# Pixel-Talk/CanonSwap

Hardware: AMD Instinct MI355X
Metric: frames/sec at 512x512 (generator hot path F->W->T->R->W->G) (higher is better)
Workload: dtype f16; 1 GPU; BASELINE configs[2]: 512x512 video, 64 frames batched per launch on each GPU, steady state over 1280 frames (20 launches per GPU) (256x256 crops in, random-init weights of the real architecture); frames_per_launch_per_gpu=64, frames_total=1280, parallelism=frame-shard x1, identities_resident=1, latency_mode=False, accumulate=fp32, debug_decodes=False

## Files before the change

canonswap_amd/csrc/conv_epilogue.h:

```cpp
#pragma once
#include "common.h"

#ifndef EP_TL
#define EP_TL(i) do { } while (0)
#endif
typedef unsigned int ep_u4_t __attribute__((ext_vector_type(4)));
typedef unsigned int ep_u2_t __attribute__((ext_vector_type(2)));

static inline int ep_check_extents(const ConvParams& p, const char* who)
{
    auto span = [&](const TDesc& t) -> long {
        return (long)(p.N - 1) * t.sN + (long)(p.D - 1) * t.sD + (long)(p.H - 1) * t.sH + (long)(p.W - 1) * t.sW + p.Cout;
    };
    auto wide = [&](const TDesc& t) { return t.sD >= (1L << 23) || t.sH >= (1L << 23) || t.sW >= (1L << 23); };
    const long lim = 1L << 31;
    long ph_max = 0;
    for (int z = 0; z < p.nphase && z < 4; ++z) ph_max = p.ph_ooff[z] > ph_max ? (long)p.ph_ooff[z] : ph_max;
    if ((p.out0.p && span(p.out0) + ph_max >= lim) || (p.out1.p && span(p.out1) >= lim) || (p.res.p && span(p.res) >= lim)) {
        cs_set_error("%s: a tensor of this launch spans 2^31 elements or more (32-bit in-tensor offsets)", who);
        return -1;
    }
    if ((p.out0.p && wide(p.out0)) || (p.out1.p && wide(p.out1)) || (p.res.p && wide(p.res)) || p.D >= (1 << 22) || p.H >= (1 << 22) ||
        p.W >= (1 << 22)) {
        cs_set_error("%s: an axis stride of 2^23 elements or more (24-bit multiplies in the addressing)", who);
// ... 78 lines not shown
__device__ __forceinline__ constexpr int ep_chan(int pair, int cstep, int wave_row0, int ci, int l4)
{
    if (pair == 1) return wave_row0 + (ci >> 1) * 32 + l4 * 8 + (ci & 1) * 4;
    if (pair == 2) return wave_row0 / 2 + (ci >> 2) * 32 + l4 * 8 + ((ci >> 1) & 1) * 4;
    const int pb = wave_row0 / 16 + ci;
    return (cstep == 2 ? (pb >> 1) : pb) * 16 + l4 * 4;
}
__device__ __forceinline__ constexpr bool ep_second(int pair, int ci) { return pair == 1 ? (ci & 1) != 0 : pair == 2 ? ((ci >> 1) & 1) != 0 : false; }
__device__ __forceinline__ bool ep_al8(const TDesc& t)
{
    return (((unsigned long long)t.p & 15ull) == 0) && (((t.sN | t.sD | t.sH | t.sW) & 7) == 0);
}
__device__ __forceinline__ constexpr int ep_pair_of(int mode, int wch)
{
    return (mode == MODE_PIXSHUF) ? 0 : (mode == MODE_TBLEND || mode == MODE_SPADE) ? (wch % 4 == 0 ? 2 : 0) : (wch % 2 == 0 ? 1 : 0);
}

#if defined(CS_EP_NOSTORE)
#define EP_STORE_COND && (p.N < 0)
#else
#define EP_STORE_COND
#endif
#define CONV_EPILOGUE_EARLY_FETCH() \
    ep_u2_t ep_xpre[EP_EARLY ? EP_WPX0 : 1][EP_EARLY ? (WCH + 1) / 2 : 1]; \
    if constexpr (EP_EARLY) { \
        int xlw, xlh, xld, xln; \
        { int t = l15p; xlw = t & mW; t >>= lgTW; xlh = t & mH; t >>= lgTH; xld = t & mD; t >>= lgTD; xln = t; } \
        const int xrs = p.res_shift, xnb = tn * (BM >> lgS); \
        const unsigned xlane = (unsigned)((xnb + xln) * (int)p.res.sN + __mul24((td << lgTD) + xld, (int)p.res.sD) + \
                                          __mul24(((th << lgTH) + xlh) >> xrs, (int)p.res.sH) + __mul24(((tw << lgTW) + xlw) >> xrs, (int)p.res.sW)); \
_Pragma("unroll") \
        for (int pi = 0; pi < EP_WPX0; ++pi) { \
            int bw, bh, bd, bn; \
            { int t = (ep_wpx0 * EP_WPX0 + pi) << 4; bw = t & mW; t >>= lgTW; bh = t & mH; t >>= lgTH; bd = t & mD; t >>= lgTD; bn = t; } \
            const unsigned xb = xlane + (unsigned)(bn * (int)p.res.sN + bd * (int)p.res.sD + (bh >> xrs) * (int)p.res.sH + (bw >> xrs) * (int)p.res.sW); \
_Pragma("unroll") \
            for (int ci = 0; ci < WCH; ci += 2) { \
                const int cb = ep_chan(EP_PAIR, 2, n0 + wch * WCH * 16, ci, l4); \
                ep_u2_t q2; q2[0] = 0u; q2[1] = 0u; \
                if (p.res.p && xnb + xln + bn < p.N && cb < p.Cout) q2 = *(const ep_u2_t*)((const half_t*)p.res.p + (xb + (unsigned)cb)); \
                ep_xpre[pi][ci / 2] = q2; \
            } \
        } \
    }

template <int N> __device__ __forceinline__ float ep_row_shl(float a)
{
#ifdef EP_HOST_EMULATION
    (void)a;
    return 0.f;
#else
    return __builtin_bit_cast(float, __builtin_amdgcn_update_dpp(0, __builtin_bit_cast(int, a), 0x100 | N, 0xf, 0xf, true));
#endif
}

__device__ __forceinline__ float ep_row_sum16(float a)
{
#ifdef EP_HOST_EMULATION
    for (int o = 1; o < 16; o <<= 1) a += __shfl_xor(a, o, 64);
    return a;
#else
    a += __builtin_bit_cast(float, __builtin_amdgcn_update_dpp(0, __builtin_bit_cast(int, a), 0x101, 0xf, 0xf, true));
    a += __builtin_bit_cast(float, __builtin_amdgcn_update_dpp(0, __builtin_bit_cast(int, a), 0x102, 0xf, 0xf, true));
    a += __builtin_bit_cast(float, __builtin_amdgcn_update_dpp(0, __builtin_bit_cast(int, a), 0x104, 0xf, 0xf, true));
    a += __builtin_bit_cast(float, __builtin_amdgcn_update_dpp(0, __builtin_bit_cast(int, a), 0x108, 0xf, 0xf, true));
    return a;
#endif
}

#define EP_STAT_FLUSH(sg) \
    if (EP_STAT) { \
        const int ep_tiles = p.nTW * p.nTH * p.nTD; \
        const int ep_nblk = EP_NBLK_V; \
        const int ep_blk = EP_BLK_V(sg); \
_Pragma("unroll") \
        for (int ci = 0; ci < WCH; ci += CSTEP) { \
            const int cb = ep_chan(EP_PAIR, CSTEP, n0 + wch * WCH * 16, ci, l4); \
            float ep_pa[4], ep_pb[4]; \
_Pragma("unroll") \
            for (int r = 0; r < 4; ++r) { \
                ep_pa[r] = ep_row_sum16(ep_sum[EP_STAT ? ci : 0][r]); ep_pb[r] = ep_row_sum16(ep_sq[EP_STAT ? ci : 0][r]); \
                ep_sum[EP_STAT ? ci : 0][r] = 0.f; ep_sq[EP_STAT ? ci : 0][r] = 0.f; \
            } \
             \
            if (l15 == 0 && cb < p.Cout) { \
                float4* dst = (float4*)(p.stat_out + (((long)tn * ep_nblk + ep_blk) * p.Cout + cb) * 2); \
                dst[0] = make_float4(ep_pa[0], ep_pb[0], ep_pa[1], ep_pb[1]); \
                dst[1] = make_float4(ep_pa[2], ep_pb[2], ep_pa[3], ep_pb[3]); \
            } \
        } \
    }

#ifndef EP_GSEL_V
#define EP_GSEL_V 0
#endif
#ifndef EP_BLK_V
#define EP_BLK_V(sg) ((tile_lin % ep_tiles) * (BM / (EP_SG * 16)) + ep_wpx * (EP_WPX / EP_SG) + (sg))
#define EP_NBLK_V (ep_tiles * (BM / (EP_SG * 16)))
#endif
#ifndef EP_SLICE_FENCE
#define EP_SLICE_FENCE
#endif
#ifndef EP_FG
#define EP_FG 8
#endif
#ifndef EP_FG_F32
#define EP_FG_F32 4
#endif
#ifndef EP_FG_STAT
#define EP_FG_STAT 4
#endif
#ifndef EP_PIPE_V
#define EP_PIPE_V 0
#endif
#ifndef EP_O0_EXTRA_V
#define EP_O0_EXTRA_V 0u
#endif
#ifndef EP_POOL_WSH_V
#define EP_POOL_WSH_V 0
#define EP_POOL_HSH_V 0
#endif
#define EP_POOLB 128
#ifndef EP_SPMUL_V
#define EP_SPMUL_V 0
#endif
#ifndef EP_O1ONLY_V
#define EP_O1ONLY_V 0
#endif
#ifndef EP_MLIN_V
#define EP_MLIN_V 0
#endif
#ifndef EP_DUP_V
#define EP_DUP_V 0
#endif
#define EP_SPMULB 256
#define EP_GELUB 512
#define EP_FETCH_ROUND(PG0, BI) \
    if (EP_PF && !EP_EARLY && (ep_fetch || ep_has_ps)) { \
_Pragma("unroll") \
        for (int g = 0; g < EP_G; ++g) { \
            int bw, bh, bd, bn; \
            { int t = (ep_wpx * EP_WPX + (PG0) + g) << 4; bw = t & mW; t >>= lgTW; bh = t & mH; t >>= lgTH; bd = t & mD; t >>= lgTD; bn = t; } \
            if (!EPFAST && ep_nb + ep_ln + bn >= p.N) continue; \
            if (ep_has_ps) ep_ps2[BI][g] = p.pixscale[ep_lane_ps + (unsigned)((((bn * p.D + bd) * p.H + bh) * p.W + bw) * p.ps_stride)]; \
            if (ep_fetch) { \
                const unsigned xb = ep_lane_res + (unsigned)(bn * (int)p.res.sN + bd * (int)p.res.sD + (bh >> ep_rs) * (int)p.res.sH + \
                                                            (bw >> ep_rs) * (int)p.res.sW); \
_Pragma("unroll") \
                for (int ci = 0; ci < WCH; ci += CSTEP) { \
                    const int cb = ep_chan(EP_PAIR, CSTEP, n0 + wch * WCH * 16, ci, l4); \
                    if (!EPALL && cb >= p.Cout) continue; \
                    if (ep_res32) ep_raw2[BI][g][(EP_PF ? ci / CSTEP : 0)] = *(const ep_u4_t*)((const float*)p.res.p + (xb + (unsigned)cb)); \
                    else if (ep_mr && ep_second(EP_PAIR, ci)) {  } \
                    else if (ep_mr && (EPALL || cb + 4 < p.Cout)) ep_raw2[BI][g][(EP_PF ? ci / CSTEP : 0)] = *(const ep_u4_t*)((const half_t*)p.res.p + (xb + (unsigned)cb)); \
                    else { \
                        const ep_u2_t q2 = *(const ep_u2_t*)((const half_t*)p.res.p + (xb + (unsigned)cb)); \
                        ep_raw2[BI][g][(EP_PF ? ci / CSTEP : 0)][0] = q2[0]; ep_raw2[BI][g][(EP_PF ? ci / CSTEP : 0)][1] = q2[1]; \
                    } \
                } \
            } \
        } \
    }
#define CONV_EPILOGUE_IMPL(EPCODE) \
    constexpr int EPF = (EPCODE); \
    constexpr bool EPFAST = EPF >= 0; \
    constexpr bool EPALL = EPFAST && ((EPF >> 6) & 1) == 0;       \
    constexpr bool EP_POOL = EPFAST && ((EPF >> 7) & 1) != 0 && (EP_POOL_WSH_V) > 0;       \
    constexpr int EP_PS = EP_POOL ? 1 : 0; \
    constexpr bool EP_GELU = EPFAST && ((EPF >> 9) & 1) != 0;           \
    const bool ep_spm = EPFAST ? (((EPF >> 8) & 1) != 0) : ((MODE == MODE_STD) && p.spmul != 0); \
    constexpr bool EP_POOL_HB = EP_POOL && (EP_POOL_HSH_V) == 0;       \
    float ep_phold[EP_POOL_HB ? WCH : 1][4];                            \
    const bool ep_has_res = EPFAST ? ((EPF & 3) != 0) : (p.res.p != nullptr); \
    const bool ep_res32 = EPFAST ? ((EPF & 3) == 2) : (p.res_f32 != 0); \
    const bool ep_has_o0 = EPFAST ? (((EPF >> 2) & 1) != 0) : (p.out0.p != nullptr); \
// ... 43 lines not shown
    { int t = l15p; ep_lw = t & mW; t >>= lgTW; ep_lh = t & mH; t >>= lgTH; ep_ld = t & mD; t >>= lgTD; ep_ln = t; } \
    const int ep_w0 = tw << lgTW, ep_h0 = th << lgTH, ep_d0 = td << lgTD, ep_nb = tn * (BM >> lgS); \
    const int ep_rs = (MODE == MODE_SPADE || ep_spm) ? p.res_shift : 0; \
     \
    const bool ep_tn1 = (BM >> lgS) == 1; \
    const unsigned ep_lane_res = (unsigned)(ep_nb * (int)p.res.sN + (ep_tn1 ? 0 : ep_ln * (int)p.res.sN) + __mul24(ep_d0 + ep_ld, (int)p.res.sD) + \
                                            __mul24((ep_h0 + ep_lh) >> ep_rs, (int)p.res.sH) + __mul24((ep_w0 + ep_lw) >> ep_rs, (int)p.res.sW)); \
    const unsigned ep_lane_o0 = (EP_O0_EXTRA_V) + (unsigned)(ep_nb * (int)p.out0.sN + (ep_tn1 ? 0 : ep_ln * (int)p.out0.sN) + __mul24(ep_d0 + ep_ld, (int)p.out0.sD) + \
                                           __mul24((ep_h0 + ep_lh) >> EP_PS, (int)p.out0.sH) + __mul24((ep_w0 + ep_lw) >> EP_PS, (int)p.out0.sW)); \
     \
    const bool ep_pool_lane = !EP_POOL || (lane & ((EP_POOL_WSH_V) | (EP_POOL_HSH_V))) == 0; \
    const unsigned ep_lane_o1 = (EP_O0_EXTRA_V) + (unsigned)(ep_nb * (int)p.out1.sN + (ep_tn1 ? 0 : ep_ln * (int)p.out1.sN) + __mul24(ep_d0 + ep_ld, (int)p.out1.sD) + \
                                           __mul24(ep_h0 + ep_lh, (int)p.out1.sH) + __mul24(ep_w0 + ep_lw, (int)p.out1.sW)); \
    const unsigned ep_lane_ps = (unsigned)(((((ep_nb + ep_ln) * p.D + ep_d0 + ep_ld) * p.H + ep_h0 + ep_lh) * p.W + ep_w0 + ep_lw) * p.ps_stride); \
     \
    const unsigned ep_lane_px = (unsigned)((((ep_nb + ep_ln) * 3) * 2 * p.H + 2 * (ep_h0 + ep_lh)) * 2 * p.W + 2 * (ep_w0 + ep_lw)); \
     \
    constexpr bool EP_PIPE = (EP_PIPE_V) != 0 && EP_G < EP_WPX; \
    ep_u4_t ep_raw2[EP_PIPE ? 2 : 1][EP_G][EP_NCI]; float ep_ps2[EP_PIPE ? 2 : 1][EP_G]; \
    if (EP_PIPE) { EP_FETCH_ROUND(0, 0) } \
_Pragma("unroll") \
    for (int pg = 0; pg < EP_WPX; pg += EP_G) { \
    const int ep_bi = EP_PIPE ? ((pg / EP_G) & 1) : 0; \
    if (!EP_PIPE) { EP_FETCH_ROUND(pg, 0) } \
    else if (pg + EP_G < EP_WPX) { EP_FETCH_ROUND(pg + EP_G, EP_PIPE ? (((pg / EP_G) + 1) & 1) : 0) } \
    ep_u4_t (&ep_raw)[EP_G][EP_NCI] = ep_raw2[ep_bi]; float (&ep_ps)[EP_G] = ep_ps2[ep_bi]; \
    if (pg == 0) EP_TL(6); \
_Pragma("unroll") \
    for (int g = 0; g < EP_G; ++g) { \
        const int pi = pg + g; \
        if (pi == 1) EP_TL(7); \
        if (pi > 0 && pi % EP_SG == 0) { EP_STAT_FLUSH(pi / EP_SG - 1) } \
        int bw, bh, bd, bn; \
        { int t = (ep_wpx * EP_WPX + pi) << 4; bw = t & mW; t >>= lgTW; bh = t & mH; t >>= lgTH; bd = t & mD; t >>= lgTD; bn = t; } \
        if (!EPFAST && ep_nb + ep_ln + bn >= p.N) continue; \
        float ps = 1.f; \
        if (ep_has_ps) ps = EP_PF ? ep_ps[g] : p.pixscale[ep_lane_ps + (unsigned)((((bn * p.D + bd) * p.H + bh) * p.W + bw) * p.ps_stride)]; \
        const unsigned xb = ep_lane_res + (unsigned)(bn * (int)p.res.sN + bd * (int)p.res.sD + (bh >> ep_rs) * (int)p.res.sH + (bw >> ep_rs) * (int)p.res.sW); \
        const unsigned ob0 = ep_lane_o0 + (unsigned)(bn * (int)p.out0.sN + bd * (int)p.out0.sD + (bh >> EP_PS) * (int)p.out0.sH + (bw >> EP_PS) * (int)p.out0.sW); \
        const unsigned ob1 = ep_lane_o1 + (unsigned)(bn * (int)p.out1.sN + bd * (int)p.out1.sD + bh * (int)p.out1.sH + bw * (int)p.out1.sW); \
        float ep_vh[4] = {0.f, 0.f, 0.f, 0.f}, ep_uh[4] = {0.f, 0.f, 0.f, 0.f};       \
_Pragma("unroll") \
        for (int ci = 0; ci < WCH; ci += CSTEP) { \
            const int cb = ep_chan(EP_PAIR, CSTEP, n0 + wch * WCH * 16, ci, l4); \
            if (!EPALL && cb >= p.Cout) continue; \
            float rr[4] = {0.f, 0.f, 0.f, 0.f};      \
            if (ep_has_res) { \
                if (EP_EARLY) { \
                    const h4_t hx = __builtin_bit_cast(h4_t, ep_xpre[EP_EARLY ? pi : 0][EP_EARLY ? ci / 2 : 0]); \
_Pragma("unroll") \
                    for (int r = 0; r < 4; ++r) rr[r] = (float)hx[r]; \
                } else if (EP_PF) { \
                    const bool ep_hi = ep_mr && ep_second(EP_PAIR, ci);       \
                    const ep_u4_t q4 = ep_raw[g][(EP_PF ? ci / CSTEP : 0)]; \
                    const ep_u4_t qp = ep_raw[g][(EP_PF && ep_second(EP_PAIR, ci) ? ci / CSTEP - 1 : 0)]; \
                    if (ep_res32) { \
                        const f4_t qf = __builtin_bit_cast(f4_t, q4);      \
_Pragma("unroll") \
                        for (int r = 0; r < 4; ++r) rr[r] = qf[r]; \
                    } else { \
                        ep_u2_t q2; q2[0] = ep_hi ? qp[2] : q4[0]; q2[1] = ep_hi ? qp[3] : q4[1]; \
                        const h4_t hx = __builtin_bit_cast(h4_t, q2); \
_Pragma("unroll") \
                        for (int r = 0; r < 4; ++r) rr[r] = (float)hx[r]; \
                    } \
                } else { \
                    load4(p.res, ep_res32, (long)(xb + (unsigned)cb), rr); \
// ... 155 lines not shown
```

canonswap_amd/csrc/conv_halo_kernel.h:

```cpp
#pragma once
#include <type_traits>
#include <utility>
#include <cstdlib>
#include "common.h"
#ifdef CS_TIMELINE
#define EP_TL(i) TL_STAMP(i)
#endif
#define EP_POOL_WSH_V EP_POOL_WSH_K
#define EP_POOL_HSH_V EP_POOL_HSH_K
#define EP_SPMUL_V EP_SPMUL_K
#define EP_DUP_V EP_DUP_K
#define EP_MLIN_V EP_MLIN_K
#define EP_O1ONLY_V EP_O1ONLY_K
#define EP_O0_EXTRA_V ep_o0_extra
#include "conv_epilogue.h"

typedef unsigned int u4_t __attribute__((ext_vector_type(4)));
__device__ __forceinline__ unsigned mdiv(unsigned u, unsigned magic) { return magic ? __umulhi(u, magic) : u; }

template <int OFF>
__device__ __forceinline__ void wfrag_load(u4_t& dst, const half_t* ptr)
{
    asm volatile("global_load_dwordx4 %0, %1, off offset:%2" : "=v"(dst) : "v"(ptr), "n"(OFF));
}
template <int N>
__device__ __forceinline__ void wait_vmcnt_le()
{
    asm volatile("s_waitcnt vmcnt(%0)" ::"n"(N) : "memory");
}

#ifdef CS_TIMELINE
extern unsigned long long* g_cs_tl;
extern long g_cs_tl_cap;
#define TL_STAMP(i) do { __builtin_amdgcn_sched_barrier(0); tl_t[i] = __builtin_amdgcn_s_memtime(); __builtin_amdgcn_sched_barrier(0); } while (0)
#else
#define TL_STAMP(i) do { } while (0)
#endif

template <int ST> struct StaticShape { static constexpr int KD = 0, KH = 0, KW = 0, LW = 0, LH = 0, LD = 0; };
template <> struct StaticShape<1> { static constexpr int KD = 1, KH = 3, KW = 3, LW = 4, LH = 3, LD = 0; };
template <> struct StaticShape<2> { static constexpr int KD = 3, KH = 3, KW = 3, LW = 3, LH = 3, LD = 1; };
template <> struct StaticShape<3> { static constexpr int KD = 3, KH = 3, KW = 3, LW = 2, LH = 2, LD = 4; };
template <> struct StaticShape<4> { static constexpr int KD = 7, KH = 7, KW = 1, LW = 3, LH = 3, LD = 1; };
template <> struct StaticShape<5> { static constexpr int KD = 3, KH = 3, KW = 3, LW = 2, LH = 2, LD = 3; };
template <> struct StaticShape<6> { static constexpr int KD = 7, KH = 7, KW = 1, LW = 1, LH = 3, LD = 3; };
template <> struct StaticShape<7> { static constexpr int KD = 3, KH = 3, KW = 3, LW = 3, LH = 3, LD = 2; };
template <> struct StaticShape<8> { static constexpr int KD = 7, KH = 7, KW = 1, LW = 1, LH = 3, LD = 4; };
// ... 9 lines not shown

template <int CK, int WPX, int WCH, int WVP, int ST, int MODE> constexpr int halo_pad()
{
#ifdef CS_LDS_V1
    return 1;
#else
    if (CK == 64 && WCH == 4 && WPX == 8 && ST == 1) return 2;
    if (CK == 32 && WCH == 5 && WPX == 8 && (ST == 7 || ST == 8 || ST == 9)) return 2;
    if (CK == 64 && WCH == 2 && WPX == 8 && WVP == 2 && ST == 16) return 2;
    if (CK == 32 && WCH == 2 && WPX == 8 && ST == 1 && MODE == MODE_SPADE) return 2;
#ifdef CS_LDS_V32
    if (CK == 32 && WCH == 2 && WPX == 4 && WVP == 4 && ST == 3) return 2;
#endif
    return 1;
#endif
}
template <int ST, int PAD> constexpr int halo_hi()
{
    if (PAD == 2) return ST == 3 ? 16 : (ST == 9 ? 19 : ((ST == 7 || ST == 8) ? 15 : (ST == 16 ? 13 : 8)));
    return ST == 4 ? 18 : ((ST == 3 || ST == 7 || ST == 8 || ST == 9) ? 13 : (ST == 12 ? 9 : 8));
}
template <int ST, int PAD> __host__ __device__ constexpr int halo_lane_pos(int l)
{
#ifdef CS_LDS_V1
    return l;
#else
    using SS = StaticShape<ST>;
    if (ST == 0 || SS::KW != 3 || SS::LW > 3 || SS::LW < 2) return l;
    if (SS::LW == 2 && PAD == 2) return ((l & 1) << 1) | ((l & 2) << 2) | ((l >> 2) & 1) | ((l & 8) >> 1);
    return ((l & 1) << 1) | ((l & 2) << 1) | ((l >> 2) & 1) | (l & 8);
#endif
}

template <class F, int... I> __device__ __forceinline__ void halo_static_for_impl(F&& f, std::integer_sequence<int, I...>) { (f(std::integral_constant<int, I>{}), ...); }
template <int N, class F> __device__ __forceinline__ void halo_static_for(F&& f) { halo_static_for_impl(static_cast<F&&>(f), std::make_integer_sequence<int, N>{}); }

template <int WCH, int PFS, int HI, int ST0>
constexpr int halo_ring_young(int st, int L, int NP, bool dma_cur)
{
    auto dma = [&](int u, bool on) { return (on && u >= ST0 && u < ST0 + HI) ? 1 : 0; };
    auto cur_before = [&](int from_step ) {
        int n = 0;
        for (int u = from_step; u < st; ++u) n += (u >= 1 ? WCH : 0) + dma(u, dma_cur);
        return n;
    };
    if (st >= PFS) {
        const int u0 = st - PFS + 1;
        return dma(u0, dma_cur) + cur_before(u0 + 1);
    }
    const int prime = (PFS - 1 - st) * WCH + cur_before(0);
    int g = 0;
    if (NP % PFS == 0) g = st + NP - PFS + 1;
    else { for (int u = NP - PFS + 1; u <= NP; ++u) if ((u - 1) % PFS == st) g = u; }
    int carried = dma(g, true);
    for (int u = g + 1; u <= NP; ++u) carried += WCH + (u < NP ? dma(u, true) : 0);
    carried += cur_before(0);
    return prime < carried ? prime : carried;
}

template <int ST, int PAD> constexpr int halo_pool_shift(int bit)
{
    for (int b = 0; b < 4; ++b) if (halo_lane_pos<ST, PAD>(1 << b) == (1 << bit)) return 1 << b;
    return 0;
}

template <int WCH, int ST> constexpr bool halo_phase_group() { return !(ST == 0 && WCH >= 4); }
// ... 41 lines not shown
    unsigned long long tl_t[8] = {0, 0, 0, 0, 0, 0, 0, 0};
    const unsigned long long tl_real0 = __builtin_amdgcn_s_memrealtime();
    TL_STAMP(0);
#endif

#ifdef CS_DEPHASE
    if (MODE == MODE_SPADE && WCH == 4) {
        unsigned hwid;
        asm volatile("s_getreg_b32 %0, hwreg(HW_REG_HW_ID)" : "=s"(hwid));
        if ((hwid & 1u) && (int)(blockIdx.x + blockIdx.y * gridDim.x) < 512)
            for (int i = 0; i < CS_DEPHASE; ++i) __builtin_amdgcn_s_sleep(16);
    }
#endif
    const int tid = threadIdx.x, lane = tid & 63;
    const int wave = __builtin_amdgcn_readfirstlane(tid >> 6);
    constexpr bool PHK = halo_phase_group<WCH, ST>();
    const int phz = (PHK && p.nphase) ? (int)blockIdx.z : 0;
    const int PHv = (PHK && p.nphase) ? p.ph_PH[phz] : p.PH, PWv = (PHK && p.nphase) ? p.ph_PW[phz] : p.PW;
    const unsigned ep_o0_extra = (PHK && p.nphase) ? p.ph_ooff[phz] : 0u;
    const int wpx = SK ? 0 : wave % WVP, wch = SK ? 0 : wave / WVP;
    const int l15 = lane & 15, l4 = lane >> 4;
    const int l15p = halo_lane_pos<ST, PAD>(l15);
#ifdef CS_NO_PAIR
    constexpr int EP_PAIR = 0;
#else
    constexpr int EP_PAIR = ep_pair_of(MODE, WCH);
#endif

#ifdef CS_NO_ASMRING
    constexpr bool ASMRK = false;
#else
    constexpr bool ASMRK = DB && !SK && CK == 32 && WCH == 5 && WPX == 8 && WVP == 2 && (ST == 7 || ST == 8 || ST == 9) && MODE == MODE_STD;
#endif
    u4_t wr_p[ASMRK ? 3 : 1][ASMRK ? WCH : 1];
    unsigned poffb[ASMRK ? HI : 1];
    __amdgpu_buffer_rsrc_t rsrc_p;
    int gbuf = 0;
    bool staged = false;
    const bool persist = ASMRK && p.persist_total > 0;
    int p_base = 0, p_cnt = 0, p_j = 0, p_i = 0, p_per = 1;
    if (persist) {
        const int total = p.persist_total, G = (int)gridDim.x;
        const int xcd = blockIdx.x & 7, q = total >> 3, r = total & 7;
        p_i = blockIdx.x >> 3; p_per = G >> 3;
        p_base = xcd * q + (xcd < r ? xcd : r); p_cnt = q + (xcd < r ? 1 : 0);
        if (p_i >= p_cnt) return;
    }
    for (;;) {
    int tile_lin = blockIdx.x, cblk = blockIdx.y;
    const bool has_next = persist && p_i + p_per * (p_j + 1) < p_cnt;
    auto u_to_tile = [&](int u, int& tl_, int& cb_) {
        const int ncb = p.Cout_pad / BN;
        tl_ = (int)mdiv((unsigned)u, p.mg_ncb); cb_ = u - tl_ * ncb;
    };
    if (persist) u_to_tile(p_base + p_i + p_per * p_j, tile_lin, cblk);
    else if (p.xcd_map != 0) {
        const int flat = p.xcd_map == 2;
        const int total = (int)gridDim.x;
        const int xcd = blockIdx.x & 7, i = blockIdx.x >> 3;
        const int q = total >> 3, r = total & 7;
        const int u = xcd * q + (xcd < r ? xcd : r) + i;
        if (flat) u_to_tile(u, tile_lin, cblk);
        else tile_lin = u;
    }
    int t = tile_lin, tq;
    tq = (int)mdiv((unsigned)t, p.mg_tw); const int tw = t - tq * p.nTW; t = tq;
// ... 46 lines not shown
    auto stage_halo = [&](int buf, int c0) {
        long coff = c0;
        int climit = p.Cin - c0;
        if ((CK == 32 || ST == 15 || (ST == 0 && WCH != 4)) && p.cg > 0) {
            const int j = c0 >> 5;
            coff = (long)(j / p.cg) * p.in_sG + (j % p.cg) * 32;
            climit = p.cg_cin - (j % p.cg) * 32;
        }
        if (pre) {
#pragma unroll
            for (int j = 0; j < HI; ++j) {
                const int q = tid + 256 * j;
                if (q < nitems) {
                    const bool ok = ((pmask >> j) & 1u) && ((q % SLP) * 8 < climit);
                    glds(ok ? p.in + poff[j] + coff : p.zero, buf, 256 * j + wave * 64);
                }
            }
        } else if constexpr (!DB) {
            for (int q0 = 0; q0 < nitems; q0 += 256) {
                const int q = q0 + tid;
                if (q < nitems) {
                    bool inb;
                    const int o = piece_off(q, inb);
                    const bool ok = inb && ((q % SLP) * 8 < climit);
                    glds(ok ? p.in + o + coff : p.zero, buf, q0 + wave * 64);
                }
            }
        }
    };

    int abase[WPX];
#pragma unroll
    for (int pi = 0; pi < WPX; ++pi) {
        int m = wpx * WPX * 16 + pi * 16 + l15p;
        const int wl = m & mW; m >>= lgTW;
        const int hl = m & mH; m >>= lgTH;
        const int dl = m & mD; m >>= lgTD;
        abase[pi] = (((m * HD + dl) * HH + hl) * HW + wl) * VS + l4 * 16;
    }
    const int nck = (p.Cin + CK - 1) / CK;
    const int j0 = SK ? wave : 0;
    int cc_lo = 0, cc_hi = nck;
    if (p.sk_out) { cc_lo = (int)(((long)nck * blockIdx.z) / gridDim.z); cc_hi = (int)(((long)nck * (blockIdx.z + 1)) / gridDim.z); }

    const half_t* wbase = p.wgt;
    if (p.wslot) wbase += p.wofs[p.wslot[nb < p.N ? nb : p.N - 1]];
    if (PHK && p.nphase) wbase += p.ph_wofs[phz];
    const half_t* wlane = wbase + ((long)(n0 + wch * WCH * 16) * 32 + ep_lane_row(EP_PAIR, l15) * 32 + l4 * 8);
    const long wstep = (long)p.Cout_pad * 32;

#ifdef CS_NO_EARLY
    constexpr bool EP_EARLY = false;
#else
    constexpr bool EP_EARLY = (MODE == MODE_SPADE) && !SK && ST != 0 && WCH == 2 && WPX == 8;
#endif
#ifdef CS_NO_EPFAST
    constexpr bool EP_FAST = false;
#else
    constexpr bool EP_FAST = !SK && ST != 0 && (WCH == 4 || WCH == 5 || (WCH == 2 && WPX == 8) || ST == 15);
#endif
    constexpr int EP_WPX0 = WPX;
    const int ep_wpx0 = wpx;
    CONV_EPILOGUE_EARLY_FETCH()

    f4_t acc[WCH][WPX];
#pragma unroll
    for (int ci = 0; ci < WCH; ++ci)
// ... 52 lines not shown
                const int climit = (nxt && !has_next) ? 0 : p.Cin - c0;
                const unsigned off = (((tid + 256 * j) % SLP) * 8 < climit) ? poffb[j] : OOB;
                __builtin_amdgcn_raw_ptr_buffer_load_lds(rsrc_p, (__attribute__((address_space(3))) void*)(smem + (size_t)buf * HSTRIDE + (size_t)(256 * j + wave * 64) * 16),
                                                         16, (int)off, c0 * 2, 0, 0);
            };
            auto wsrc_of = [&](int cc, int st, int nsc) -> const half_t* {
                int c2 = cc, s2 = st;
                if (st >= nsc) { c2 = cc + 1; s2 = (nsc % PFS == 0) ? st - nsc : (st - PFS) % PFS; }
                const int ccl = c2 < cc_hi ? c2 : cc_lo;
                return wlane + (long)(ccl * NT + s2) * wstep;
            };
            auto wload1 = [&](u4_t& dst, const half_t* src, int ci) {
                if (ci == 0) asm volatile("global_load_dwordx4 %0, %1, off" : "=v"(dst) : "v"(src));
                else if (ci == 1) asm volatile("global_load_dwordx4 %0, %1, off offset:1024" : "=v"(dst) : "v"(src));
                else if (ci == 2) asm volatile("global_load_dwordx4 %0, %1, off offset:2048" : "=v"(dst) : "v"(src));
                else if (ci == 3) asm volatile("global_load_dwordx4 %0, %1, off offset:3072" : "=v"(dst) : "v"(src));
                else asm volatile("global_load_dwordx4 %0, %1, off" : "=v"(dst) : "v"(src + 4 * 16 * 32));
            };
            static_assert(EP_PAIR == 0, "ASMR: plain weight row order");
            TL_STAMP(1);
            constexpr bool CARRY = ST != 9;
            if (!staged) {
                set_stage(nb, d0, h0, w0);
#pragma unroll
                for (int j = 0; j < HI; ++j) stage_piece(gbuf, cc_lo, j);
            }
            if (!staged || !CARRY) {
#pragma unroll
                for (int st = 0; st < PFS; ++st)
#pragma unroll
                    for (int ci = 0; ci < WCH; ++ci) wload1(wr[st][ci], wsrc_of(cc_lo, st, NS), ci);
            }
            TL_STAMP(2);
            auto run_chunk_a = [&](int cc, auto rag_t) {
                constexpr bool RAG = decltype(rag_t)::value;
                wait_vmcnt_le<PFS * WCH>();
                __builtin_amdgcn_s_barrier();
                asm volatile("" ::: "memory");
                const unsigned char* hb = smem + (size_t)gbuf * HSTRIDE;
                const int nbuf = gbuf ^ 1;
                gbuf ^= 1;
                if (cc + 1 == cc_hi && has_next) {
                    int ntl, ncb_, t2 = 0, q2;
                    u_to_tile(p_base + p_i + p_per * (p_j + 1), ntl, ncb_);
                    t2 = ntl;
                    q2 = (int)mdiv((unsigned)t2, p.mg_tw); const int tw2 = t2 - q2 * p.nTW; t2 = q2;
                    q2 = (int)mdiv((unsigned)t2, p.mg_th); const int th2 = t2 - q2 * p.nTH; t2 = q2;
                    q2 = (int)mdiv((unsigned)t2, p.mg_td); const int td2 = t2 - q2 * p.nTD; t2 = q2;
                    set_stage(t2 * TN, td2 << lgTD, th2 << lgTH, tw2 << lgTW);
                }
                constexpr int HA = WPX / 2;
                constexpr int PK = SS::KW > 1 ? SS::KW : SS::KH, SPR = PK / 2 + PK % 2;
                constexpr int NSC = RAG ? (NT / PK) * SPR : NS;
                auto tap_of = [&](int st) -> int { return RAG ? (st / SPR) * PK + 2 * (st % SPR) : st; };
                auto paired = [&](int st) -> bool { return RAG && (st % SPR) < PK / 2; };
                auto toff_of = [&](int st) -> int {
                    const int tap = tap_of(st);
                    return (((tap / (SS::KW * SS::KH)) * SHH + (tap / SS::KW) % SS::KH) * SHW + tap % SS::KW) * VS;
                };
                int abP[RAG ? WPX : 1];
                if constexpr (RAG) {
                    const int pd = (l4 >= 2) ? (SS::KW > 1 ? VS : SHW * VS) - 32 : 0;
#pragma unroll
                    for (int pi = 0; pi < WPX; ++pi) abP[pi] = abase[pi] + pd;
                }
                auto ab_of = [&](int pi, int st) -> int { return paired(st) ? abP[RAG ? pi : 0] : abase[pi]; };
                h8_t afA[HA], afB[WPX - HA];
#pragma unroll
                for (int pi = 0; pi < HA; ++pi) afA[pi] = *(const h8_t*)(hb + ab_of(pi, 0) + toff_of(0));
                halo_static_for<NSC>([&](auto stc) {
                    constexpr int st = decltype(stc)::value;
                    {
#ifdef CS_ASMR_DEBUG0
                        constexpr int NY = 0;
#else
                        constexpr int NY = halo_ring_young<WCH, PFS, HI, ST0>(st, NSC, NS, true);
#endif
                        asm volatile("s_waitcnt vmcnt(%5)" : "+v"(wr[st % PFS][0]), "+v"(wr[st % PFS][1]), "+v"(wr[st % PFS][2]), "+v"(wr[st % PFS][3]),
                                                             "+v"(wr[st % PFS][4]) : "n"(NY));
                    }
                    __builtin_amdgcn_sched_barrier(0);
                    const half_t* rsrc_w = wsrc_of(cc, st - 1 + PFS, NSC);
                    const int toff = toff_of(st);
#pragma unroll
                    for (int k = 0; k < 2 * WCH; ++k) {
                        const int ci = k >> 1, p0 = (k & 1) * 2;
                        acc[ci][p0] = __builtin_amdgcn_mfma_f32_16x16x32_f16(__builtin_bit_cast(h8_t, wr[st % PFS][ci]), afA[p0], acc[ci][p0], 0, 0, 0);
                        acc[ci][p0 + 1] = __builtin_amdgcn_mfma_f32_16x16x32_f16(__builtin_bit_cast(h8_t, wr[st % PFS][ci]), afA[p0 + 1], acc[ci][p0 + 1], 0, 0, 0);
                        if (k >= 2 && k < 6) afB[k - 2] = *(const h8_t*)(hb + ab_of(HA + k - 2, st) + toff);
                        if constexpr (st >= 1) { if (k >= 5) wload1(wr[(st - 1) % PFS][k - 5], rsrc_w, k - 5); }
                        __builtin_amdgcn_sched_barrier(0);
                    }
                    if (st >= ST0 && st < ST0 + HI) { stage_piece(nbuf, cc + 1, st - ST0); __builtin_amdgcn_sched_barrier(0); }
#pragma unroll
                    for (int k = 0; k < 2 * WCH; ++k) {
                        const int ci = k >> 1, p0 = (k & 1) * 2;
                        acc[ci][HA + p0] = __builtin_amdgcn_mfma_f32_16x16x32_f16(__builtin_bit_cast(h8_t, wr[st % PFS][ci]), afB[p0], acc[ci][HA + p0], 0, 0, 0);
                        acc[ci][HA + p0 + 1] = __builtin_amdgcn_mfma_f32_16x16x32_f16(__builtin_bit_cast(h8_t, wr[st % PFS][ci]), afB[p0 + 1], acc[ci][HA + p0 + 1], 0, 0, 0);
                        if (k >= 2 && k < 6 && st + 1 < NSC) afA[k - 2] = *(const h8_t*)(hb + ab_of(k - 2, st + 1) + toff_of(st + 1));
                        __builtin_amdgcn_sched_barrier(0);
                    }
                });
                {
                    const half_t* rsrc_w = wsrc_of(cc, NSC - 1 + PFS, NSC);
#pragma unroll
                    for (int ci = 0; ci < WCH; ++ci) wload1(wr[(NSC - 1) % PFS][ci], rsrc_w, ci);
                }
            };
            const bool rag = RAGK && p.ragged && cc_hi == nck;
            for (int cc = cc_lo; cc < cc_hi - (rag ? 1 : 0); ++cc) run_chunk_a(cc, std::false_type{});
            if constexpr (RAGK) {
                if (rag) run_chunk_a(cc_hi - 1, std::true_type{});
            }
            staged = has_next;
            if (!has_next || !CARRY) {
                wait_vmcnt_le<0>();
                __builtin_amdgcn_sched_barrier(0);
            }
#pragma unroll
            for (int st = 0; st < PFS; ++st)
                asm volatile("" :: "v"(wr[st][0]), "v"(wr[st][1]), "v"(wr[st][2]), "v"(wr[st][3]), "v"(wr[st][4]));
        } else {
        u4_t wr[PFS][WCH];
        auto wload_at = [&](u4_t (&dst)[WCH], int cc, int st) {
            const int ccl = cc < nck ? cc : nck - 1;
            const half_t* src = wlane + (long)((ccl * KH32 + st % KH32) * NT + st / KH32) * wstep;
#pragma unroll
            for (int ci = 0; ci < WCH; ++ci) dst[ci] = *(const u4_t*)(src + ep_frag_row(EP_PAIR, ci) * 32);
        };
        TL_STAMP(1);
        stage_halo(0, cc_lo * CK);
        __syncthreads();
        TL_STAMP(2);
        if (DB && cc_lo + 1 < cc_hi) stage_halo(1, (cc_lo + 1) * CK);
        auto chunk_head = [&](int cc) -> const unsigned char* {
// ... 165 lines not shown
                if (done) break;
                while (ctap < C.tap) { ++ctap; if (++ckw == KW) { ckw = 0; if (++ckh == KH) { ckh = 0; ++ckd; } } }
                const int toff = ((ckd * HH + ckh) * HW + ckw) * VS + C.half * 64;
                h8_t af[WPX];
    #pragma unroll
                for (int pi = 0; pi < WPX; ++pi) af[pi] = *(const h8_t*)(hb + abase[pi] + toff);
                wait_vmcnt_le<WCH*(PFD - 1)>();
                __builtin_amdgcn_sched_barrier(0);
    #pragma unroll
                for (int ci = 0; ci < WCH; ++ci)
    #pragma unroll
                    for (int pi = 0; pi < WPX; ++pi)
                        acc[ci][pi] = __builtin_amdgcn_mfma_f32_16x16x32_f16(__builtin_bit_cast(h8_t, wr[i][ci]), af[pi], acc[ci][pi], 0, 0, 0);
                __builtin_amdgcn_sched_barrier(0);
                wload(wr[i]);
                it_advance(C);
            }
        }
    }

    if constexpr (ST == 0) {
        wait_vmcnt_le<0>();
        __builtin_amdgcn_sched_barrier(0);
    }

    constexpr bool EP_HEAVY = (MODE == MODE_PIXSHUF) || (WCH == 1) || (ST == 15) || (ST == 0);
    constexpr bool KWSUM = !SK && MODE == MODE_STD && WCH == 5 && WPX == 8 && WVP == 2 && (ST == 8 || ST == 9);
    TL_STAMP(3);
    if constexpr (!SK) {
        if (p.sk_out) {
            const long mtot = (long)p.N * p.D * p.H * p.W;
#pragma unroll
            for (int pi = 0; pi < WPX; ++pi) {
                int m = wpx * WPX * 16 + pi * 16 + l15p;
                const int w = (tw << lgTW) + (m & mW); m >>= lgTW;
                const int h = (th << lgTH) + (m & mH); m >>= lgTH;
                const int d = (td << lgTD) + (m & mD); m >>= lgTD;
                const int n = tn * TN + m;
                if (n >= p.N) continue;
                const long pos = (((long)n * p.D + d) * p.H + h) * p.W + w;
#pragma unroll
                for (int ci = 0; ci < WCH; ++ci)
                    *(f4_t*)(p.sk_out + ((long)blockIdx.z * mtot + pos) * p.Cout_pad + ep_chan(EP_PAIR, 1, n0 + wch * WCH * 16, ci, l4)) = acc[ci][pi];
            }
        } else if (XSK && p.xs_w) {
            if constexpr (XSK) {
                __syncthreads();
                float* part = (float*)smem;
                const int cw0 = n0 + wch * 64;
                h8_t wsA[4][2];
#pragma unroll
                for (int of = 0; of < 4; ++of)
#pragma unroll
                    for (int q = 0; q < 2; ++q)
                        wsA[of][q] = *(const h8_t*)(p.xs_w + ((long)((cw0 >> 5) + q) * 64 + of * 16 + l15) * 32 + l4 * 8);
                float gb[2][8], mu[2][8], rs[2][8];
#pragma unroll
                for (int q = 0; q < 2; ++q) {
                    const int cb = cw0 + q * 32 + l4 * 8;
#pragma unroll
                    for (int j = 0; j < 8; j += 4) {
                        const float4 b4 = p.bias ? *(const float4*)(p.bias + cb + j) : make_float4(0.f, 0.f, 0.f, 0.f);
                        gb[q][j] = b4.x; gb[q][j + 1] = b4.y; gb[q][j + 2] = b4.z; gb[q][j + 3] = b4.w;
                        const float4 q0 = *(const float4*)(p.stats + ((long)tn * p.Cout + cb + j) * 2);
                        const float4 q1 = *(const float4*)(p.stats + ((long)tn * p.Cout + cb + j) * 2 + 4);
                        mu[q][j] = q0.x; rs[q][j] = q0.y; mu[q][j + 1] = q0.z; rs[q][j + 1] = q0.w;
                        mu[q][j + 2] = q1.x; rs[q][j + 2] = q1.y; mu[q][j + 3] = q1.z; rs[q][j + 3] = q1.w;
// ... 58 lines not shown
#pragma unroll
                        for (int r = 0; r < 4; ++r) sum[r] += (float)br[r];
                        ep_u2_t o2; o2[0] = ep_pk(sum[0], sum[1]); o2[1] = ep_pk(sum[2], sum[3]);
                        *(ep_u2_t*)((half_t*)p.xs_out.p + po) = o2;
                    }
                    xr[0] = xn[0]; xr[1] = xn[1]; br = bn;
                }
            }
        } else if (KWSUM && p.kw_out) {
            if constexpr (KWSUM && ST == 9) {
                __syncthreads();
                constexpr int ZERO = 16 * 160;
                float* buf = (float*)(smem + (ASMRK ? (size_t)(gbuf ^ 1) * (HI * 4096) : 0)) + wpx * (16 * 160 + 4);
                const int th128 = wch * 64 + lane;
                if (th128 == 0) buf[ZERO] = 0.f;
                int offT[2][4][4]; int goff[2]; bool on[2];
#pragma unroll
                for (int q = 0; q < 2; ++q) {
                    const int fi = q * 128 + th128;
                    on[q] = fi < 220;
                    const int fic = on[q] ? fi : 0;
                    goff[q] = (fic / 55) * (p.nTW * 220) + (fic % 55) * 4;
#pragma unroll
                    for (int e = 0; e < 4; ++e) {
                        const int idx = (fic % 55) * 4 + e, c = idx % 22, j = idx / 22, h = fic / 55;
#pragma unroll
                        for (int t = 0; t < 4; ++t) {
                            const int kw = t + 6 - j;
                            offT[q][e][t] = (kw >= 0 && kw <= 6) ? ((h << 2) | t) * 160 + kw * 22 + c : ZERO;
                        }
                    }
                }
                const long gslice = (long)p.H * p.nTW * 220;
                float* const gbase = p.kw_out + ((((long)tn * p.D + (td << lgTD) + wpx * 4) * p.H + (th << lgTH)) * p.nTW + tw) * 220;
#pragma unroll
                for (int pi = 0; pi < WPX; ++pi) {
#pragma unroll
                    for (int ci = 0; ci < WCH; ++ci) *(f4_t*)(buf + l15p * 160 + wch * (WCH * 16) + ci * 16 + l4 * 4) = acc[ci][pi];
                    __syncthreads();
#pragma unroll
                    for (int q = 0; q < 2; ++q) {
                        if (on[q]) {
                            f4_t v;
#pragma unroll
                            for (int e = 0; e < 4; ++e) v[e] = ((buf[offT[q][e][0]] + buf[offT[q][e][1]]) + buf[offT[q][e][2]]) + buf[offT[q][e][3]];
                            *(f4_t*)(gbase + (pi >> 1) * gslice + (long)(pi & 1) * 4 * (p.nTW * 220) + goff[q]) = v;
                        }
                    }
                    __syncthreads();
                }
            } else if constexpr (KWSUM) {
                __syncthreads();
                constexpr int ZERO = 16 * 160;
                float* buf = (float*)(smem + (ASMRK ? (size_t)(gbuf ^ 1) * (HI * 4096) : 0)) + wpx * (16 * 160 + 4);
                const int th128 = wch * 64 + lane;
                if (th128 == 0) buf[ZERO] = 0.f;
                int offA[12], offB[12], goff[3];
#pragma unroll
                for (int q = 0; q < 3; ++q) {
                    const int fi = q * 128 + th128;
                    goff[q] = (fi * 4 / 176) * (p.nTW * 176) + (fi * 4) % 176;
#pragma unroll
                    for (int e = 0; e < 4; ++e) {
                        const int idx = fi * 4 + e, c = idx % 22, j = (idx / 22) & 7, h = (idx / 176) & 7;
                        offA[q * 4 + e] = j <= 6 ? (h << 1) * 160 + (6 - j) * 22 + c : ZERO;
                        offB[q * 4 + e] = j >= 1 ? ((h << 1) | 1) * 160 + (7 - j) * 22 + c : ZERO;
                    }
                }
                float* const gbase = p.kw_out + ((((long)tn * p.D + (td << lgTD) + wpx * WPX) * p.H + (th << lgTH)) * p.nTW + tw) * 176;
                const long gslice = (long)p.H * p.nTW * 176;
#pragma unroll
                for (int pi = 0; pi < WPX; ++pi) {
#pragma unroll
                    for (int ci = 0; ci < WCH; ++ci) *(f4_t*)(buf + l15p * 160 + wch * (WCH * 16) + ci * 16 + l4 * 4) = acc[ci][pi];
                    __syncthreads();
#pragma unroll
                    for (int q = 0; q < 3; ++q) {
                        if (q * 128 + th128 < 352) {
                            f4_t v;
// ... 223 lines not shown
```

Before: 537.9 frames/s.

## Interleave halo conv pixel blocks across waves and skip MFMAs on padded depth faces

For the ASMR halo conv kernels (stride 7/9 variants), pixel blocks are now dealt round-robin between the two pixel waves instead of contiguously. Each wave then holds blocks from every depth slice, and at the depth boundary the MFMAs and A-fragment loads for taps that fall in zero padding are skipped with a scalar branch. The epilogue, split-K and kw-sum store addressing are remapped to the new block order. This removes wasted matrix work on edge tiles at the cost of inline-asm branches, extra s_nops and more complex addressing, and it risks correctness if the remapping is incomplete.

```diff
diff --git a/canonswap_amd/csrc/conv_epilogue.h b/canonswap_amd/csrc/conv_epilogue.h
--- a/canonswap_amd/csrc/conv_epilogue.h
+++ b/canonswap_amd/csrc/conv_epilogue.h
@@ -134,7 +134,7 @@
 _Pragma("unroll") \
         for (int pi = 0; pi < EP_WPX0; ++pi) { \
             int bw, bh, bd, bn; \
-            { int t = (ep_wpx0 * EP_WPX0 + pi) << 4; bw = t & mW; t >>= lgTW; bh = t & mH; t >>= lgTH; bd = t & mD; t >>= lgTD; bn = t; } \
+            { int t = EP_BLOCK_V(ep_wpx0, EP_WPX0, pi) << 4; bw = t & mW; t >>= lgTW; bh = t & mH; t >>= lgTH; bd = t & mD; t >>= lgTD; bn = t; } \
             const unsigned xb = xlane + (unsigned)(bn * (int)p.res.sN + bd * (int)p.res.sD + (bh >> xrs) * (int)p.res.sH + (bw >> xrs) * (int)p.res.sW); \
 _Pragma("unroll") \
             for (int ci = 0; ci < WCH; ci += 2) { \
@@ -193,6 +193,9 @@
         } \
     }
 
+#ifndef EP_BLOCK_V
+#define EP_BLOCK_V(w, W, pi) ((w) * (W) + (pi))
+#endif
 #ifndef EP_GSEL_V
 #define EP_GSEL_V 0
 #endif
@@ -242,7 +245,7 @@
 _Pragma("unroll") \
         for (int g = 0; g < EP_G; ++g) { \
             int bw, bh, bd, bn; \
-            { int t = (ep_wpx * EP_WPX + (PG0) + g) << 4; bw = t & mW; t >>= lgTW; bh = t & mH; t >>= lgTH; bd = t & mD; t >>= lgTD; bn = t; } \
+            { int t = EP_BLOCK_V(ep_wpx, EP_WPX, (PG0) + g) << 4; bw = t & mW; t >>= lgTW; bh = t & mH; t >>= lgTH; bd = t & mD; t >>= lgTD; bn = t; } \
             if (!EPFAST && ep_nb + ep_ln + bn >= p.N) continue; \
             if (ep_has_ps) ep_ps2[BI][g] = p.pixscale[ep_lane_ps + (unsigned)((((bn * p.D + bd) * p.H + bh) * p.W + bw) * p.ps_stride)]; \
             if (ep_fetch) { \
@@ -352,7 +355,7 @@
         if (pi == 1) EP_TL(7); \
         if (pi > 0 && pi % EP_SG == 0) { EP_STAT_FLUSH(pi / EP_SG - 1) } \
         int bw, bh, bd, bn; \
-        { int t = (ep_wpx * EP_WPX + pi) << 4; bw = t & mW; t >>= lgTW; bh = t & mH; t >>= lgTH; bd = t & mD; t >>= lgTD; bn = t; } \
+        { int t = EP_BLOCK_V(ep_wpx, EP_WPX, pi) << 4; bw = t & mW; t >>= lgTW; bh = t & mH; t >>= lgTH; bd = t & mD; t >>= lgTD; bn = t; } \
         if (!EPFAST && ep_nb + ep_ln + bn >= p.N) continue; \
         float ps = 1.f; \
         if (ep_has_ps) ps = EP_PF ? ep_ps[g] : p.pixscale[ep_lane_ps + (unsigned)((((bn * p.D + bd) * p.H + bh) * p.W + bw) * p.ps_stride)]; \
diff --git a/canonswap_amd/csrc/conv_halo_kernel.h b/canonswap_amd/csrc/conv_halo_kernel.h
--- a/canonswap_amd/csrc/conv_halo_kernel.h
+++ b/canonswap_amd/csrc/conv_halo_kernel.h
@@ -13,6 +13,7 @@
 #define EP_MLIN_V EP_MLIN_K
 #define EP_O1ONLY_V EP_O1ONLY_K
 #define EP_O0_EXTRA_V ep_o0_extra
+#define EP_BLOCK_V(w, W, pi) (halo_block<W, DEALK>(w, pi))
 #include "conv_epilogue.h"
 
 typedef unsigned int u4_t __attribute__((ext_vector_type(4)));
@@ -88,6 +89,16 @@
 #endif
 }
 
+template <int WPX, bool DEAL> __host__ __device__ constexpr int halo_block(int wpx, int pi) { return DEAL ? pi * 2 + wpx : wpx * WPX + pi; }
+template <int CK, int WPX, int WCH, int WVP, int MODE, bool DB, bool SK, int ST> constexpr bool halo_deal()
+{
+#ifdef CS_NO_ASMRING
+    return false;
+#else
+    return DB && !SK && CK == 32 && WCH == 5 && WPX == 8 && WVP == 2 && (ST == 7 || ST == 9) && MODE == MODE_STD;
+#endif
+}
+
 template <class F, int... I> __device__ __forceinline__ void halo_static_for_impl(F&& f, std::integer_sequence<int, I...>) { (f(std::integral_constant<int, I>{}), ...); }
 template <int N, class F> __device__ __forceinline__ void halo_static_for(F&& f) { halo_static_for_impl(static_cast<F&&>(f), std::make_integer_sequence<int, N>{}); }
 
@@ -195,6 +206,8 @@
 #else
     constexpr bool ASMRK = DB && !SK && CK == 32 && WCH == 5 && WPX == 8 && WVP == 2 && (ST == 7 || ST == 8 || ST == 9) && MODE == MODE_STD;
 #endif
+    constexpr bool DEALK = halo_deal<CK, WPX, WCH, WVP, MODE, DB, SK, ST>();
+    static_assert(!DEALK || ASMRK, "the dealt block map belongs to the ASMR kernels");
     u4_t wr_p[ASMRK ? 3 : 1][ASMRK ? WCH : 1];
     unsigned poffb[ASMRK ? HI : 1];
     __amdgpu_buffer_rsrc_t rsrc_p;
@@ -307,7 +320,7 @@
     int abase[WPX];
 #pragma unroll
     for (int pi = 0; pi < WPX; ++pi) {
-        int m = wpx * WPX * 16 + pi * 16 + l15p;
+        int m = halo_block<WPX, DEALK>(wpx, pi) * 16 + l15p;
         const int wl = m & mW; m >>= lgTW;
         const int hl = m & mH; m >>= lgTH;
         const int dl = m & mD; m >>= lgTD;
@@ -426,6 +439,11 @@
                     for (int ci = 0; ci < WCH; ++ci) wload1(wr[st][ci], wsrc_of(cc_lo, st, NS), ci);
             }
             TL_STAMP(2);
+            int edge = 0;
+            if constexpr (DEALK) {
+                const bool lo = d0 == 0, hi = d0 + (1 << SS::LD) == p.D;
+                edge = (p.PD == SS::KD / 2 && lo != hi) ? (lo ? 1 : 2) : 0;
+            }
             auto run_chunk_a = [&](int cc, auto rag_t) {
                 constexpr bool RAG = decltype(rag_t)::value;
                 wait_vmcnt_le<PFS * WCH>();
@@ -459,9 +477,27 @@
                     for (int pi = 0; pi < WPX; ++pi) abP[pi] = abase[pi] + pd;
                 }
                 auto ab_of = [&](int pi, int st) -> int { return paired(st) ? abP[RAG ? pi : 0] : abase[pi]; };
+                auto pad_face = [&](int pi, int st) -> int {
+                    const int pl = ((halo_block<WPX, DEALK>(0, pi) << 4) >> (SS::LW + SS::LH)) + tap_of(st) / (SS::KW * SS::KH) - SS::KD / 2;
+                    return !DEALK ? 0 : (pl < 0 ? 1 : (pl >= (1 << SS::LD) ? 2 : 0));
+                };
+                auto runs = [&](int face) -> bool { return face == 0 || edge != face; };
+                auto mfma_unless = [&](int face, f4_t& c, const u4_t& w, const h8_t& a) __attribute__((always_inline)) {
+                    if (face == 1) asm volatile("s_cmp_eq_u32 %3, 1\n\ts_cbranch_scc1 .Lhalo_pad%=\n\tv_mfma_f32_16x16x32_f16 %0, %1, %2, %0\n.Lhalo_pad%=:" : "+a"(c) : "v"(w), "v"(a), "s"(edge) : "scc");
+                    else asm volatile("s_cmp_eq_u32 %3, 2\n\ts_cbranch_scc1 .Lhalo_pad%=\n\tv_mfma_f32_16x16x32_f16 %0, %1, %2, %0\n.Lhalo_pad%=:" : "+a"(c) : "v"(w), "v"(a), "s"(edge) : "scc");
+                };
+                auto mfma_unless2 = [&](int face, f4_t& c0, f4_t& c1, const u4_t& w, const h8_t& a0, const h8_t& a1) __attribute__((always_inline)) {
+                    if (face == 1) asm volatile("s_cmp_eq_u32 %5, 1\n\ts_cbranch_scc1 .Lhalo_pad%=\n\tv_mfma_f32_16x16x32_f16 %0, %2, %3, %0\n\tv_mfma_f32_16x16x32_f16 %1, %2, %4, %1\n.Lhalo_pad%=:" : "+a"(c0), "+a"(c1) : "v"(w), "v"(a0), "v"(a1), "s"(edge) : "scc");
+                    else asm volatile("s_cmp_eq_u32 %5, 2\n\ts_cbranch_scc1 .Lhalo_pad%=\n\tv_mfma_f32_16x16x32_f16 %0, %2, %3, %0\n\tv_mfma_f32_16x16x32_f16 %1, %2, %4, %1\n.Lhalo_pad%=:" : "+a"(c0), "+a"(c1) : "v"(w), "v"(a0), "v"(a1), "s"(edge) : "scc");
+                };
+                auto mfma_pair = [&](int f0, int f1, f4_t& c0, f4_t& c1, const u4_t& w, const h8_t& a0, const h8_t& a1) __attribute__((always_inline)) {
+                    if (f0 != 0 && f0 == f1) { mfma_unless2(f0, c0, c1, w, a0, a1); return; }
+                    if (f0 == 0) c0 = __builtin_amdgcn_mfma_f32_16x16x32_f16(__builtin_bit_cast(h8_t, w), a0, c0, 0, 0, 0); else mfma_unless(f0, c0, w, a0);
+                    if (f1 == 0) c1 = __builtin_amdgcn_mfma_f32_16x16x32_f16(__builtin_bit_cast(h8_t, w), a1, c1, 0, 0, 0); else mfma_unless(f1, c1, w, a1);
+                };
                 h8_t afA[HA], afB[WPX - HA];
 #pragma unroll
-                for (int pi = 0; pi < HA; ++pi) afA[pi] = *(const h8_t*)(hb + ab_of(pi, 0) + toff_of(0));
+                for (int pi = 0; pi < HA; ++pi) if (runs(pad_face(pi, 0))) afA[pi] = *(const h8_t*)(hb + ab_of(pi, 0) + toff_of(0));
                 halo_static_for<NSC>([&](auto stc) {
                     constexpr int st = decltype(stc)::value;
                     {
@@ -479,9 +515,9 @@
 #pragma unroll
                     for (int k = 0; k < 2 * WCH; ++k) {
                         const int ci = k >> 1, p0 = (k & 1) * 2;
-                        acc[ci][p0] = __builtin_amdgcn_mfma_f32_16x16x32_f16(__builtin_bit_cast(h8_t, wr[st % PFS][ci]), afA[p0], acc[ci][p0], 0, 0, 0);
-                        acc[ci][p0 + 1] = __builtin_amdgcn_mfma_f32_16x16x32_f16(__builtin_bit_cast(h8_t, wr[st % PFS][ci]), afA[p0 + 1], acc[ci][p0 + 1], 0, 0, 0);
-                        if (k >= 2 && k < 6) afB[k - 2] = *(const h8_t*)(hb + ab_of(HA + k - 2, st) + toff);
+                        const int f0 = pad_face(p0, st), f1 = pad_face(p0 + 1, st);
+                        mfma_pair(f0, f1, acc[ci][p0], acc[ci][p0 + 1], wr[st % PFS][ci], afA[p0], afA[p0 + 1]);
+                        if (k >= 2 && k < 6 && runs(pad_face(HA + k - 2, st))) afB[k - 2] = *(const h8_t*)(hb + ab_of(HA + k - 2, st) + toff);
                         if constexpr (st >= 1) { if (k >= 5) wload1(wr[(st - 1) % PFS][k - 5], rsrc_w, k - 5); }
                         __builtin_amdgcn_sched_barrier(0);
                     }
@@ -489,12 +525,13 @@
 #pragma unroll
                     for (int k = 0; k < 2 * WCH; ++k) {
                         const int ci = k >> 1, p0 = (k & 1) * 2;
-                        acc[ci][HA + p0] = __builtin_amdgcn_mfma_f32_16x16x32_f16(__builtin_bit_cast(h8_t, wr[st % PFS][ci]), afB[p0], acc[ci][HA + p0], 0, 0, 0);
-                        acc[ci][HA + p0 + 1] = __builtin_amdgcn_mfma_f32_16x16x32_f16(__builtin_bit_cast(h8_t, wr[st % PFS][ci]), afB[p0 + 1], acc[ci][HA + p0 + 1], 0, 0, 0);
-                        if (k >= 2 && k < 6 && st + 1 < NSC) afA[k - 2] = *(const h8_t*)(hb + ab_of(k - 2, st + 1) + toff_of(st + 1));
+                        const int f0 = pad_face(HA + p0, st), f1 = pad_face(HA + p0 + 1, st);
+                        mfma_pair(f0, f1, acc[ci][HA + p0], acc[ci][HA + p0 + 1], wr[st % PFS][ci], afB[p0], afB[p0 + 1]);
+                        if (k >= 2 && k < 6 && st + 1 < NSC && runs(pad_face(k - 2, st + 1))) afA[k - 2] = *(const h8_t*)(hb + ab_of(k - 2, st + 1) + toff_of(st + 1));
                         __builtin_amdgcn_sched_barrier(0);
                     }
                 });
+                if constexpr (DEALK) asm volatile("s_nop 7\n\ts_nop 7" ::: "memory");
                 {
                     const half_t* rsrc_w = wsrc_of(cc, NSC - 1 + PFS, NSC);
 #pragma unroll
@@ -726,7 +763,7 @@
             const long mtot = (long)p.N * p.D * p.H * p.W;
 #pragma unroll
             for (int pi = 0; pi < WPX; ++pi) {
-                int m = wpx * WPX * 16 + pi * 16 + l15p;
+                int m = halo_block<WPX, DEALK>(wpx, pi) * 16 + l15p;
                 const int w = (tw << lgTW) + (m & mW); m >>= lgTW;
                 const int h = (th << lgTH) + (m & mH); m >>= lgTH;
                 const int d = (td << lgTD) + (m & mD); m >>= lgTD;
@@ -851,9 +888,11 @@
                     }
                 }
                 const long gslice = (long)p.H * p.nTW * 220;
-                float* const gbase = p.kw_out + ((((long)tn * p.D + (td << lgTD) + wpx * 4) * p.H + (th << lgTH)) * p.nTW + tw) * 220;
+                const int bwv = halo_block<WPX, DEALK>(wpx, 0);
+                float* const gbase = p.kw_out + ((((long)tn * p.D + (td << lgTD) + (bwv >> 1)) * p.H + (th << lgTH) + (bwv & 1) * 4) * p.nTW + tw) * 220;
 #pragma unroll
                 for (int pi = 0; pi < WPX; ++pi) {
+                    const int bpi = halo_block<WPX, DEALK>(0, pi);
 #pragma unroll
                     for (int ci = 0; ci < WCH; ++ci) *(f4_t*)(buf + l15p * 160 + wch * (WCH * 16) + ci * 16 + l4 * 4) = acc[ci][pi];
                     __syncthreads();
@@ -863,7 +902,7 @@
                             f4_t v;
 #pragma unroll
                             for (int e = 0; e < 4; ++e) v[e] = ((buf[offT[q][e][0]] + buf[offT[q][e][1]]) + buf[offT[q][e][2]]) + buf[offT[q][e][3]];
-                            *(f4_t*)(gbase + (pi >> 1) * gslice + (long)(pi & 1) * 4 * (p.nTW * 220) + goff[q]) = v;
+                            *(f4_t*)(gbase + (bpi >> 1) * gslice + (long)(bpi & 1) * 4 * (p.nTW * 220) + goff[q]) = v;
                         }
                     }
                     __syncthreads();
```

After: 530.3 frames/s. 0.986x the previous value.
